# peterWon/GLoc3D

Hardware: AMD Instinct MI355X
Metric: localization queries/sec (kNN+top-20 reg), KITTI-00-sized DB (higher is better)
Workload: dtype f32

## Files before the change

gloc3d_amd/csrc/common.hip:

```cpp
#include "common.hpp"

namespace gloc {

char* err_buf() {
  static thread_local char buf[512] = {0};
  return buf;
}

void set_err(const char* fmt, ...) {
  va_list ap;
  va_start(ap, fmt);
  vsnprintf(err_buf(), 512, fmt, ap);
  va_end(ap);
}

int select_device(int device) {
  int n = 0;
  hipError_t e = hipGetDeviceCount(&n);
  if (e != hipSuccess || n <= 0) {
    set_err("no HIP device visible (%s): the gloc3d hot path has no CPU fallback",
            e == hipSuccess ? "device count 0" : hipGetErrorString(e));
    return GLOC_ERR_NODEVICE;
  }
  if (device < 0 || device >= n) {
    set_err("device ordinal %d out of range [0,%d)", device, n);
    return GLOC_ERR_INVALID;
  }
  hipDeviceProp_t prop;
  GLOC_HIP(hipGetDeviceProperties(&prop, device));
  if (strncmp(prop.gcnArchName, "gfx950", 6) != 0) {
    set_err("device %d is %s; this library is built for gfx950 (MI355X) only", device,
            prop.gcnArchName);
    return GLOC_ERR_NODEVICE;
  }
  GLOC_HIP(hipSetDevice(device));
  return GLOC_OK;
}

int DevBuf::ensure(size_t bytes, hipStream_t s, bool keep, size_t used) {
  if (bytes <= cap) return GLOC_OK;
  size_t ncap = cap ? cap : 256;
  while (ncap < bytes) ncap += ncap / 2 + 256;
  void* np = nullptr;
  GLOC_HIP(hipMalloc(&np, ncap));
  if (keep && p && used) {
    hipError_t e = hipMemcpyAsync(np, p, used, hipMemcpyDeviceToDevice, s);
    if (e == hipSuccess) e = hipStreamSynchronize(s);
    if (e != hipSuccess) {
      (void)hipFree(np);
      set_err("device buffer growth failed: %s", hipGetErrorString(e));
      return GLOC_ERR_HIP;
    }
  }
  if (p) GLOC_HIP(hipFree(p));
  p = np;
  cap = ncap;
  return GLOC_OK;
}

void DevBuf::release() {
  if (p) (void)hipFree(p);
  p = nullptr;
  cap = 0;
}

hipEvent_t Profiler::get_event() {
  if (!pool.empty()) {
    hipEvent_t e = pool.back();
    pool.pop_back();
    return e;
  }
  hipEvent_t e;
  (void)hipEventCreate(&e);
  return e;
}

void Profiler::begin(const char* name, hipStream_t s) {
  Family& f = fam[name];
  Span sp{get_event(), get_event()};
  (void)hipEventRecord(sp.a, s);
  f.open.push_back(sp);
}

void Profiler::end(const char* name, hipStream_t s) {
  Family& f = fam[name];
  if (f.open.empty()) return;
  (void)hipEventRecord(f.open.back().b, s);
  f.launches++;
  size_t live = 0;
  for (auto& kv : fam) live += kv.second.open.size();
  if (live > 8192) (void)collect(s);
}

int Profiler::collect(hipStream_t s) {
  GLOC_HIP(hipStreamSynchronize(s));
  for (auto& kv : fam) {
    for (Span& sp : kv.second.open) {
      float ms = 0.f;
      if (hipEventElapsedTime(&ms, sp.a, sp.b) == hipSuccess) kv.second.total_ms += ms;
      pool.push_back(sp.a);
      pool.push_back(sp.b);
    }
    kv.second.open.clear();
  }
  return GLOC_OK;
}

void Profiler::reset() {
  for (auto& kv : fam) {
    for (Span& sp : kv.second.open) {
      pool.push_back(sp.a);
      pool.push_back(sp.b);
    }
    kv.second.open.clear();
    kv.second.total_ms = 0;
    kv.second.launches = 0;
  }
}

void Profiler::destroy() {
  reset();
  for (hipEvent_t e : pool) (void)hipEventDestroy(e);
  pool.clear();
  fam.clear();
}

Handle::~Handle() {
  prof.destroy();
  if (own_stream) (void)hipStreamDestroy(own_stream);
}

int handle_open(Handle* h, int device) {
  h->device = device;
  hipError_t e = hipStreamCreateWithFlags(&h->own_stream, hipStreamNonBlocking);
  if (e != hipSuccess) {
    set_err("hipStreamCreate failed: %s", hipGetErrorString(e));
    return GLOC_ERR_HIP;
  }
  h->stream = h->own_stream;
  return GLOC_OK;
}

int handle_set_stream(Handle* h, void* hip_stream) {
  GLOC_TRY(handle_synchronize(h));
  h->stream = hip_stream ? static_cast<hipStream_t>(hip_stream) : h->own_stream;
  return GLOC_OK;
}

int handle_synchronize(Handle* h) {
  GLOC_REQUIRE(h, GLOC_ERR_INVALID, "handle is NULL");
  GLOC_HIP(hipSetDevice(h->device));
  GLOC_HIP(hipStreamSynchronize(h->stream));
  return GLOC_OK;
}

int handle_set_profile(Handle* h, int enable) {
  GLOC_REQUIRE(h, GLOC_ERR_INVALID, "handle is NULL");
  h->prof.enabled = enable != 0;
  return GLOC_OK;
}

int handle_profile(Handle* h, const char* kernel, double* total_ms, uint64_t* launches) {
  GLOC_REQUIRE(h && kernel, GLOC_ERR_INVALID, "NULL argument");
  GLOC_HIP(hipSetDevice(h->device));
  GLOC_TRY(h->prof.collect(h->stream));
  auto it = h->prof.fam.find(kernel);
  if (total_ms) *total_ms = it == h->prof.fam.end() ? 0.0 : it->second.total_ms;
// ... 26 lines not shown
```

gloc3d_amd/csrc/common.hpp:

```cpp
#pragma once
#include <hip/hip_runtime.h>

#include <cstdarg>
#include <cstdint>
#include <cstdio>
#include <cstring>
#include <map>
#include <new>
#include <string>
#include <type_traits>
#include <vector>

#include "../../include/gloc3d.h"

namespace gloc {

char* err_buf();
void set_err(const char* fmt, ...);

#define GLOC_HIP(expr)                                                                    \
  do {                                                                                    \
    hipError_t e_ = (expr);                                                               \
    if (e_ != hipSuccess) {                                                               \
      ::gloc::set_err("%s failed: %s (%s:%d)", #expr, hipGetErrorString(e_), __FILE__,    \
// ... 7 lines not shown
    if (!(cond)) {                     \
      ::gloc::set_err(__VA_ARGS__);    \
      return (code);                   \
    }                                  \
  } while (0)

#define GLOC_TRY(expr)            \
  do {                            \
    int rc_ = (expr);             \
    if (rc_ != GLOC_OK) return rc_; \
  } while (0)

int select_device(int device);

struct DevBuf {
  void* p = nullptr;
  size_t cap = 0;
  DevBuf() = default;
  DevBuf(const DevBuf&) = delete;
  DevBuf& operator=(const DevBuf&) = delete;
  DevBuf(DevBuf&& o) noexcept : p(o.p), cap(o.cap) { o.p = nullptr, o.cap = 0; }
  DevBuf& operator=(DevBuf&& o) noexcept {
    if (this != &o) {
      release();
      p = o.p, cap = o.cap;
      o.p = nullptr, o.cap = 0;
    }
    return *this;
  }
  ~DevBuf() { release(); }
  int ensure(size_t bytes, hipStream_t s, bool keep = false, size_t used = 0);
  void release();
  template <class T>
  T* as() const {
    return reinterpret_cast<T*>(p);
  }
};

static_assert(!std::is_copy_constructible<DevBuf>::value && !std::is_copy_assignable<DevBuf>::value,
              "a DevBuf has one owner: two copies would free the same memory");

struct Profiler {
  bool enabled = false;
  struct Span {
    hipEvent_t a, b;
  };
  struct Family {
    std::vector<Span> open;
    double total_ms = 0;
    uint64_t launches = 0;
  };
  std::map<std::string, Family> fam;
  std::vector<hipEvent_t> pool;
  hipEvent_t get_event();
  void begin(const char* name, hipStream_t s);
  void end(const char* name, hipStream_t s);
  int collect(hipStream_t s);
  void reset();
  void destroy();
};

struct ProfScope {
  Profiler& p;
  const char* name;
  hipStream_t s;
  ProfScope(Profiler& p_, const char* n, hipStream_t s_) : p(p_), name(n), s(s_) {
    if (p.enabled) p.begin(name, s);
  }
  ~ProfScope() {
    if (p.enabled) p.end(name, s);
  }
};

struct Handle {
  int device = 0;
  hipStream_t own_stream = nullptr, stream = nullptr;
  Profiler prof;
  Handle() = default;
  Handle(const Handle&) = delete;
  Handle& operator=(const Handle&) = delete;
  ~Handle();
};

int handle_open(Handle* h, int device);
int handle_set_stream(Handle* h, void* hip_stream);
int handle_synchronize(Handle* h);
int handle_set_profile(Handle* h, int enable);
int handle_profile(Handle* h, const char* kernel, double* total_ms, uint64_t* launches);
int handle_profile_reset(Handle* h);

template <class H>
int create_handle(int device, H** out) {
  GLOC_REQUIRE(out, GLOC_ERR_INVALID, "out is NULL");
  *out = nullptr;
  GLOC_TRY(select_device(device));
  H* h = new (std::nothrow) H();
  GLOC_REQUIRE(h, GLOC_ERR_NOMEM, "out of host memory");
  const int rc = handle_open(h, device);
  if (rc != GLOC_OK) {
    delete h;
    return rc;
  }
  *out = h;
  return GLOC_OK;
}

template <class H>
int destroy_handle(H* h) {
  if (!h) return GLOC_OK;
  (void)hipSetDevice(h->device);
  (void)hipStreamSynchronize(h->stream);
  delete h;
  return GLOC_OK;
}

template <class W>
int ensure_ws(W** slot) {
  if (!*slot) *slot = new (std::nothrow) W;
  GLOC_REQUIRE(*slot, GLOC_ERR_NOMEM, "host allocation failed");
  return GLOC_OK;
}

struct Staging {
// ... 15 lines not shown
```

gloc3d_amd/csrc/nn_compact.hpp:

```cpp
#pragma once
#include <hip/hip_runtime.h>
#include <stdint.h>

#include <type_traits>

#include "lane_ops.hpp"
#include "reg_kernels.hpp"

namespace gloc {
namespace reg {

typedef float f32x2 __attribute__((ext_vector_type(2)));

#define GPTR(T) const T __attribute__((address_space(1)))*
#define CPTR(T) const T __attribute__((address_space(4)))*
constexpr float NN_NEAR = 1.0e-6f;
constexpr float NN_LB_SCALE = 0.999998f;
#ifndef GLOC_NN_THIN_MIN
#define GLOC_NN_THIN_MIN 32
#endif
#ifdef GLOC_NN_MARKS
#define NN_MARK(n) asm volatile("; NN_MARK " n)
#else
#define NN_MARK(n)
// ... 1163 lines not shown
    static_assert(ACC_NV == 18, "16 scattered moments, the d2 sum, sum |p'|^2");
    static_assert(sizeof(double) * ACC_NV >= sizeof(float) * WAVE_PARTIAL_FLOATS, "a wave partial fits a partial's slot");
    float* out = reinterpret_cast<float*>(partials + ((size_t)job * n_part + gi) * ACC_NV);
#pragma unroll
    for (int k = 0; k < 8; ++k) mv[k] = exchange_add<32>(mv[k], mv[k + 8]);
#pragma unroll
    for (int k = 0; k < 4; ++k) mv[k] = exchange_add<16>(mv[k], mv[k + 4]);
    {
      const bool up = (lane & 8) != 0;
#pragma unroll
      for (int k = 0; k < 2; ++k) {
        const float keep = up ? mv[k + 2] : mv[k], send = up ? mv[k] : mv[k + 2];
        mv[k] = keep + xor_lane<8>(send);
      }
    }
    {
      const bool up = (lane & 4) != 0;
      const float keep = up ? mv[1] : mv[0], send = up ? mv[0] : mv[1];
      mv[0] = keep + xor_lane<4>(send);
    }
    float x = mv[0], y = mv[16];
    x += xor_lane<2>(x);
    x += xor_lane<1>(x);
    y = exchange_add<32>(y, pp);
    y = exchange_add<16>(y, y);
    y += xor_lane<8>(y);
    y += xor_lane<4>(y);
    y += xor_lane<2>(y);
    y += xor_lane<1>(y);
    if ((lane & 3) == 0) st_f32<CHAIN>(out + ((lane >> 2) & 15), x);
    if (lane == 0) {
      st_f32<CHAIN>(out + 16, y);
      st_f32<CHAIN>(out + 17, cen[0]);
      st_f32<CHAIN>(out + 18, cen[1]);
      st_f32<CHAIN>(out + 19, cen[2]);
    }
    if (lane == 32) st_f32<CHAIN>(out + 20, y);
  }
  NN_MARK("end");
}

#define NN_COMPACT_PARAMS                                                                                              \
  const Job *__restrict__ jobs, uint32_t n_jobs, uint32_t job_group, uint32_t n_wg, uint32_t subs,                     \
      const CandState *__restrict__ states, const uint32_t *prev_corr, uint32_t *corr, float *__restrict__ d2out,      \
      f32x4 *__restrict__ pairs, double *__restrict__ partials, uint32_t n_part, size_t ld, float gate2, NnSplit sp,   \
      NnHeavy hv, unsigned long long *__restrict__ stat_pairs
#define NN_COMPACT_ARGS jobs, n_jobs, job_group, n_wg, subs, states, prev_corr, corr, d2out, pairs, partials, n_part, ld, gate2, sp, hv, stat_pairs

template <int CS, bool PAIRS, bool SPLIT = false, bool WARM = false>
__global__ __launch_bounds__(64 * NN_WPB) void nn_compact_kernel(NN_COMPACT_PARAMS) {
  nn_compact_body<CS, PAIRS, SPLIT, WARM>(NnPos{blockIdx.z, blockIdx.x, blockIdx.y}, NN_COMPACT_ARGS);
}

template <int CS, bool PAIRS>
__global__ __launch_bounds__(64) void nn_compact_heavy_kernel(NN_COMPACT_PARAMS) {
  nn_compact_body<CS, PAIRS, true, false, true>(NnPos{0u, 0u, 0u}, NN_COMPACT_ARGS);
}

template <int CS>
__global__ __launch_bounds__(64 * NN_WPB) __attribute__((amdgpu_waves_per_eu(6, 6))) void nn_compact_split_warm_kernel(NN_COMPACT_PARAMS) {
  nn_compact_body<CS, false, true, true>(NnPos{blockIdx.z, blockIdx.x, blockIdx.y}, NN_COMPACT_ARGS);
}

template <int CS>
__global__ __launch_bounds__(64 * NN_WPB) __attribute__((amdgpu_waves_per_eu(6, 6))) void nn_chain_kernel(NN_COMPACT_PARAMS, NnChain ch) {
  static_assert(NN_WPB == 1, "a work-group is a wave: the roles and the arrival counts are per wave");
  const uint32_t b = blockIdx.x;
  const uint32_t pass = b / ch.pass_size, r1 = b - pass * ch.pass_size;
  const uint32_t grp = r1 / ch.grp_size, r2 = r1 - grp * ch.grp_size;
  const uint32_t n_search = job_group * n_wg;
  if (r2 >= n_search) {
    const uint32_t si = r2 - n_search, jl = si / NN_CHAIN_ROLES, role = si - jl * NN_CHAIN_ROLES;
    const uint32_t job = grp * ch.jobs_per_grp + jl;
    if (jl >= ch.jobs_per_grp || job >= n_jobs) return;
    const size_t cell = ((size_t)pass * n_jobs + job) * NN_CHAIN_PAD;
    if (role == NN_CHAIN_RED) {
      if (!chain_wait<false>(ch.done + cell, ch.expected, ch.err)) return;
      if ((threadIdx.x & 63) == 0) st_u32<true>(ch.go + cell, 1u);
    } else if (!chain_wait<false>(ch.go + cell, 1u, ch.err)) {
      return;
    }
    nn_compact_body<CS, false, true, true, false, true>(NnPos{0u, 0u, 0u, 1u + role, pass, job}, jobs, n_jobs, job_group, n_wg, subs, states,
                                                        corr, corr, d2out, pairs, partials, n_part, ld, gate2, sp, hv, stat_pairs, ch);
    return;
  }
  const uint32_t wgv = r2 / job_group, slot = r2 - wgv * job_group;
  uint32_t vin = slot;
  if ((job_group & 7u) == 0u) vin = (slot & ~7u) | ((slot - (slot >> 3) - grp) & 7u);
  const uint32_t vjob = grp * job_group + vin;
  if (vjob >= n_jobs * subs) return;
  const uint32_t job = vjob / subs;
  const size_t cell = ((size_t)pass * n_jobs + job) * NN_CHAIN_PAD;
  NnSplit spp = sp;
  if (pass > 0u) {
    if (!chain_wait<true>(ch.ready + cell, 2u, ch.err)) return;
    spp.plan = ch.planp + (size_t)(pass - 1u) * n_jobs * n_part;
    spp.helper = ch.helperp + (size_t)(pass - 1u) * n_jobs * sp.hx;
  }
  nn_compact_body<CS, false, true, true, false, true>(NnPos{grp, slot, wgv, 0u, pass, job}, jobs, n_jobs, job_group, n_wg, subs, states, corr, corr,
                                                      d2out, pairs, partials, n_part, ld, gate2, spp, hv, stat_pairs, ch);
  __builtin_amdgcn_s_waitcnt(0);
  asm volatile("" ::: "memory");
  if ((threadIdx.x & 63) == 0) (void)__hip_atomic_fetch_add(ch.done + cell, 1u, __ATOMIC_RELAXED, __HIP_MEMORY_SCOPE_AGENT);
}
#undef NN_COMPACT_PARAMS
#undef NN_COMPACT_ARGS
// ... 4 lines not shown
```

gloc3d_amd/csrc/reg.hip:

```cpp
#include <algorithm>
#include <cmath>
#include <vector>

#include "common.hpp"

#include "fpfh.hpp"
#include "ndt.hpp"
#include "nn_compact.hpp"
#include "gicp.hpp"
#include "p2l.hpp"
#include "pairgraph.hpp"
#include "reg_kernels.hpp"
#include "robust.hpp"
#include "scan_store.hpp"
#include "vgicp.hpp"

using namespace gloc;
using namespace gloc::reg;

struct gloc_reg : Handle {
  hipEvent_t done_ev = nullptr;
  gloc_scan_store* store = nullptr;
  gloc_scan_store* own_store = nullptr;
  DevBuf jobs, states;
// ... 167 lines not shown
  sp.thresh = h->nn_split_thresh_set || !chained ? h->nn_split_thresh : 85000u;
  return GLOC_OK;
}

int setup_heavy(gloc_reg* h, const BatchDims& bd, int cs) {
  h->heavy = NnHeavy{};
  if (h->nn_mode == 1 || cs != 2 || h->nn_heavy_thresh <= 0) return GLOC_OK;
  const size_t cap = std::min<size_t>((size_t)bd.n_jobs * 16, 16384), S = 64 * (size_t)cs;
  hipStream_t s = h->stream;
  auto keys_at = [](size_t c) { return (256 + c * 8 + c * 4 + 255) & ~(size_t)255; };
  if (cap > h->heavy_cap) {
    GLOC_TRY(h->heavy_buf.ensure(keys_at(cap) + 2 * cap * S * 8 + 256, s));
    GLOC_HIP(hipMemsetAsync(h->heavy_buf.p, 0, keys_at(cap), s));
    GLOC_HIP(hipMemsetAsync(h->heavy_buf.as<char>() + keys_at(cap), 0xFF, cap * S * 8, s));
    h->heavy_cap = cap;
  }
  char* b = h->heavy_buf.as<char>();
  NnHeavy& hv = h->heavy;
  hv.count = reinterpret_cast<uint32_t*>(b);
  hv.list = reinterpret_cast<uint32_t*>(b + 256);
  hv.ticket = reinterpret_cast<uint32_t*>(b + 256 + h->heavy_cap * 8);
  hv.skey = reinterpret_cast<unsigned long long*>(b + keys_at(h->heavy_cap));
  hv.hkey = hv.skey + h->heavy_cap * S;
  hv.cap = (uint32_t)cap;
  hv.thresh = (uint32_t)h->nn_heavy_thresh;
  return GLOC_OK;
}

void launch_order(const gloc_reg* h, uint32_t n_jobs, uint32_t& jg, uint32_t& subs) {
  subs = h->nn_sub_jobs > 0 ? (uint32_t)h->nn_sub_jobs : (n_jobs < 48 ? 8u : 1u);
  jg = (uint32_t)h->nn_job_group;
  if (h->nn_sub_jobs > 0 || h->nn_job_group_set || n_jobs >= 48) return;
  jg = 8u;
  subs = n_jobs % 4u == 0u ? 2u : (n_jobs % 2u == 0u ? 4u : 8u);
}

struct NnArgs {
  const WsView& v;
  const BatchDims& bd;
  uint32_t jg, n_wg, subs;
  float gate2;
  unsigned long long* stat_pairs;
};

template <auto KERNEL, typename... Chain>
void launch_compact(const NnArgs& a, dim3 grid, const uint32_t* prev_corr, bool pairs, NnHeavy hv, Chain... chain) {
  hipLaunchKernelGGL(KERNEL, grid, dim3(64 * NN_WPB), 0, a.v.s, a.v.jobs, a.v.n_jobs, a.jg, a.n_wg, a.subs, a.v.states, prev_corr,
                     a.v.corr, a.v.d2, a.v.pairs, pairs ? (double*)nullptr : a.v.partials, a.bd.n_part, a.bd.ld, a.gate2, a.v.split, hv,
                     a.stat_pairs, chain...);
}

template <int CS, bool PAIRS, bool WARM>
void launch_pass(const NnArgs& a, dim3 grid, const uint32_t* prev_corr, NnHeavy hv) {
  if (!a.v.split.hx) launch_compact<nn_compact_kernel<CS, PAIRS, false, WARM>>(a, grid, prev_corr, PAIRS, hv);
  else if constexpr (CS == 2 && !PAIRS && WARM) launch_compact<nn_compact_split_warm_kernel<2>>(a, grid, prev_corr, PAIRS, hv);
  else launch_compact<nn_compact_kernel<CS, PAIRS, true, WARM>>(a, grid, prev_corr, PAIRS, hv);
}

template <int CS>
void launch_kind(const NnArgs& a, dim3 grid, const uint32_t* prev_corr, NnHeavy hv, bool want_pairs, bool warm) {
  if (want_pairs) launch_pass<CS, true, false>(a, grid, prev_corr, hv);
  else if (warm) launch_pass<CS, false, true>(a, grid, prev_corr, hv);
  else launch_pass<CS, false, false>(a, grid, prev_corr, hv);
}

int launch_nn(gloc_reg* h, const BatchDims& bd, const WsView& v, bool warm, bool want_pairs, float gate2) {
  ProfScope ps(h->prof, "nn", v.s);
  Profiler no_prof;
  ProfScope ps_cold((want_pairs || !warm) ? h->prof : no_prof, "nn_cold", v.s);
  h->nn_launches++;
  if (h->nn_mode == 1) {
    dim3 grid((bd.max_src + 256 * NN_S - 1) / (256 * NN_S), v.n_jobs);
    hipLaunchKernelGGL(nn_kernel, grid, dim3(256), 0, v.s, v.jobs, v.states,
                       v.corr, v.d2, bd.ld);
    if (want_pairs)
      hipLaunchKernelGGL(gather_pairs_kernel, dim3((bd.max_src + 255) / 256, v.n_jobs), dim3(256), 0, v.s,
                         v.jobs, v.states, v.corr, bd.ld,
                         v.pairs);
  } else {
    const int cs = h->nn_src_per_lane;
    const bool cold = want_pairs || !warm;
    const NnHeavy hv = cold ? v.heavy : NnHeavy{};
    if (hv.cap) GLOC_HIP(hipMemsetAsync(hv.count, 0, 4, v.s));
    const uint32_t n_wg_job = (bd.max_groups + v.split.hx + NN_WPB - 1) / NN_WPB;
    uint32_t jg, subs;
    launch_order(h, v.n_jobs, jg, subs);
    const uint32_t n_slots = v.n_jobs * subs;
    const uint32_t n_wg = (n_wg_job + subs - 1) / subs;
    const unsigned grid = n_wg * jg * ((n_slots + jg - 1) / jg);
    GLOC_REQUIRE(n_wg <= 65535u && (n_slots + jg - 1) / jg <= 65535u, GLOC_ERR_INVALID,
                 "the culled search's grid: %u work-groups per job slot (scans above ~8 M points) or %u job groups exceed 65535", n_wg,
                 (n_slots + jg - 1) / jg);
    if (grid) {
      const NnArgs a{v, bd, jg, n_wg, subs, gate2, h->prof.enabled ? h->counters.as<unsigned long long>() : nullptr};
      const dim3 g3(jg, n_wg, (n_slots + jg - 1) / jg);
      const uint32_t* prev_corr = warm ? v.corr : nullptr;
      if (cs == 1) launch_kind<1>(a, g3, prev_corr, hv, want_pairs, warm);
      else if (cs == 2) launch_kind<2>(a, g3, prev_corr, hv, want_pairs, warm);
      else launch_kind<4>(a, g3, prev_corr, hv, want_pairs, warm);
      if (hv.cap) {
        const dim3 gh(hv.cap * NN_HEAVY_PARTS);
        if (want_pairs) launch_compact<nn_compact_heavy_kernel<2, true>>(a, gh, nullptr, true, hv);
        else launch_compact<nn_compact_heavy_kernel<2, false>>(a, gh, nullptr, false, hv);
      }
    }
  }
  GLOC_HIP(hipGetLastError());
  return GLOC_OK;
}

bool batch_chains(const gloc_reg* h, const BatchDims& bd, uint32_t hx, uint32_t warm_passes) {
  if (!h->nn_chain || h->chain_broken || h->nn_mode == 1 || h->nn_src_per_lane != 2 || h->prof.enabled || NN_WPB != 1) return false;
  if (hx == 0 || warm_passes < 2) return false;
  uint32_t jg, subs;
  launch_order(h, bd.n_jobs, jg, subs);
  if (bd.n_jobs >= 48 || (jg & 7u) || jg % subs) return false;
  if ((bd.n_part & 31u) || (hx & 31u)) return false;
  const uint32_t n_wg = ((bd.max_groups + hx + NN_WPB - 1) / NN_WPB + subs - 1) / subs;
  const uint32_t groups = (bd.n_jobs * subs + jg - 1) / jg;
  const uint64_t grp_size = ((uint64_t)jg * n_wg + (jg / subs) * NN_CHAIN_ROLES + 7) & ~7ull;
  return grp_size * groups * warm_passes < (1ull << 31);
}
// ... 102 lines not shown
  v.jobs = h->jobs.as<Job>();
  v.states = h->states.as<CandState>();
  v.partials = h->partials.as<double>();
  if (sp.search) {
    if (!h->counters.p) {
      GLOC_TRY(h->counters.ensure(8 * NN_STAT_SLOTS, s));
      GLOC_HIP(hipMemsetAsync(h->counters.p, 0, 8 * NN_STAT_SLOTS, s));
    }
    GLOC_TRY(h->corr.ensure(sizeof(uint32_t) * std::max<size_t>(bd.ld, 1) * n_jobs, s));
    GLOC_TRY(h->d2.ensure(sizeof(float) * std::max<size_t>(bd.ld, 1) * n_jobs, s));
    v.corr = h->corr.as<uint32_t>();
    v.d2 = h->d2.as<float>();
  }
  if (sp.pairs) {
    GLOC_TRY(h->pairs.ensure(sizeof(f32x4) * 2 * bd.ld * n_jobs, s));
    GLOC_TRY(h->Rt.ensure(sizeof(float) * 12 * sp.hyp * n_jobs, s));
    GLOC_TRY(h->valid.ensure(sizeof(uint32_t) * sp.hyp * n_jobs, s));
    GLOC_TRY(h->inliers.ensure(sizeof(uint32_t) * sp.hyp * n_jobs, s));
    v.pairs = h->pairs.as<f32x4>();
    v.Rt = h->Rt.as<float>();
    v.valid = h->valid.as<uint32_t>();
    v.inliers = h->inliers.as<uint32_t>();
    if (sp.alive) {
      GLOC_TRY(h->alive.ensure(sizeof(uint32_t) * (sp.hyp + 1) * n_jobs, s));
      v.a_idx = h->alive.as<uint32_t>();
      v.a_cnt = v.a_idx + sp.hyp * n_jobs;
    }
  }
  GLOC_HIP(hipMemcpyAsync(v.jobs, h->h_jobs, sizeof(Job) * n_jobs, hipMemcpyHostToDevice, s));
  GLOC_HIP(hipMemcpyAsync(v.states, h->h_states, sizeof(CandState) * n_jobs, hipMemcpyHostToDevice, s));
  b.chained = batch_chains(h, bd, sp.split_hx, sp.warm_passes);
  GLOC_TRY(setup_split(h, bd, cs, sp.split_hx, b.chained));
  if (sp.search) GLOC_TRY(setup_heavy(h, bd, cs));
  else h->heavy = NnHeavy{};
  v.split = h->split;
  v.heavy = h->heavy;
  if (sp.search) {
    h->last_ld = bd.ld;
    h->last_jobs = n_jobs;
  }
  return GLOC_OK;
}

uint32_t score_chunk_len(uint32_t n_jobs, uint32_t max_src) {
  static_assert(1024 % SC_STAGE == 0 && SC_CHUNK % SC_STAGE == 0, "whole tiles");
  return (size_t)n_jobs * ((max_src + SC_CHUNK - 1) / SC_CHUNK) >= 2048 ? (uint32_t)SC_CHUNK : 1024u;
}

uint32_t score_hpb(uint32_t len) { return len <= 16 ? 16u : (len <= 64 ? 64u : 256u); }

int enqueue_refit(gloc_reg* h, const BatchDims& bd, const WsView& v, float thr2, uint32_t nblocks) {
  const uint32_t n_jobs = v.n_jobs;
  {
    ProfScope ps(h->prof, "accum", v.s);
    hipLaunchKernelGGL(accum_kernel<1>, dim3(nblocks, n_jobs), dim3(ACC_THREADS), 0, v.s, v.jobs, v.states, v.corr, v.d2, v.pairs, bd.ld, thr2,
                       v.partials, bd.n_part);
    GLOC_HIP(hipGetLastError());
  }
  {
    ProfScope ps(h->prof, "solve", v.s);
    hipLaunchKernelGGL(solve_kernel<1>, dim3(v.split.hx ? 2 * n_jobs : n_jobs), dim3(SOLVE_THREADS), 0, v.s, v.partials, bd.n_part, false, v.jobs,
                       v.states, v.split, n_jobs);
    GLOC_HIP(hipGetLastError());
  }
  return GLOC_OK;
}

struct RansacRule {
  uint32_t iters;
  float inlier_thresh, min_inlier_ratio, confidence;
  uint64_t seed;
};

int enqueue_ransac(gloc_reg* h, const BatchDims& bd, const RansacRule& r, const WsView& v, uint32_t nblocks) {
  const uint32_t n_jobs = v.n_jobs;
  hipStream_t s = v.s;
  const uint32_t H = r.iters;
  const bool adaptive = r.confidence > 0.f && r.confidence < 1.f;
  uint32_t bounds[4] = {0u, 0u, 0u, 0u};
  int n_ph = 0;
  for (uint32_t b : {adaptive ? 16u : 256u, adaptive ? 64u : H, H})
    if (b <= H && b > bounds[n_ph]) bounds[++n_ph] = b;
  if (bounds[n_ph] < H) bounds[++n_ph] = H;
  GLOC_HIP(hipMemsetAsync(v.valid, 0, sizeof(uint32_t) * (size_t)H * n_jobs, s));
  GLOC_HIP(hipMemsetAsync(v.inliers, 0, sizeof(uint32_t) * (size_t)H * n_jobs, s));
  const float thr2 = r.inlier_thresh * r.inlier_thresh;
  const uint32_t chunk_len = score_chunk_len(n_jobs, bd.max_src);
  const unsigned cchunks = (bd.max_src + chunk_len - 1) / chunk_len;
  for (int ph = 0; ph < n_ph; ++ph) {
    const uint32_t h0 = bounds[ph], h1 = bounds[ph + 1], len = h1 - h0;
    const CandState* st = ph ? v.states : (const CandState*)nullptr;
    {
      ProfScope ps(h->prof, "ransac_hyp", s);
      hipLaunchKernelGGL(ransac_hyp_kernel, dim3((len + 127) / 128, n_jobs), dim3(128), 0, s, v.pairs, bd.ld,
                         v.jobs, r.seed, H, h0, h1, st, v.Rt, v.valid);
      GLOC_HIP(hipGetLastError());
    }
    ProfScope ps(h->prof, "ransac_score", s);
    const uint32_t hpb = score_hpb(len);
    const unsigned NP = 8;
    if (!adaptive && ph > 0 && len >= 512 && cchunks >= NP) {
      uint32_t* a_idx = v.a_idx;
      uint32_t* a_cnt = v.a_cnt;
      for (unsigned q = 0; q < NP; ++q) {
        const unsigned c0 = q * cchunks / NP, c1 = (q + 1) * cchunks / NP;
        hipLaunchKernelGGL(ransac_alive_kernel, dim3(n_jobs), dim3(1024), 0, s, v.inliers, v.valid,
                           H, h0, h1, v.jobs, v.states, (uint32_t)(c0 * chunk_len), a_idx, a_cnt);
        hipLaunchKernelGGL(ransac_score_kernel, dim3((len + 255) / 256, c1 - c0, n_jobs), dim3(256), 0, s,
                           v.pairs, bd.ld, v.jobs, H, h0, 256u, v.Rt,
                           v.valid, thr2, st, v.inliers, a_idx, a_cnt, (uint32_t)c0, chunk_len);
      }
    } else {
      hipLaunchKernelGGL(ransac_score_kernel, dim3((len + hpb - 1) / hpb, cchunks, n_jobs), dim3(256), 0, s,
                         v.pairs, bd.ld, v.jobs, H, h0, hpb, v.Rt,
                         v.valid, thr2, st, v.inliers, (const uint32_t*)nullptr,
                         (const uint32_t*)nullptr, 0u, chunk_len);
    }
    if (ph + 1 < n_ph)
      hipLaunchKernelGGL(ransac_scan_kernel<false>, dim3(n_jobs), dim3(64), 0, s, v.inliers,
                         v.valid, v.Rt, H, h0, h1, v.jobs, r.confidence,
                         r.min_inlier_ratio, v.states);
    else
      hipLaunchKernelGGL(ransac_scan_kernel<true>, dim3(n_jobs), dim3(64), 0, s, v.inliers,
                         v.valid, v.Rt, H, h0, h1, v.jobs, r.confidence,
                         r.min_inlier_ratio, v.states);
    GLOC_HIP(hipGetLastError());
  }
  return enqueue_refit(h, bd, v, thr2, nblocks);
}

int enqueue_pipeline(gloc_reg* h, const BatchDims& bd, const gloc_reg_params* prm, const WsView& v, bool can, bool any_tgt,
                     uint32_t nblocks, bool chained) {
  const uint32_t n_jobs = v.n_jobs;
  hipStream_t s = v.s;
  const bool culled = h->nn_mode != 1;
  const float gate2 = prm->max_corr_dist > 0.f ? prm->max_corr_dist * prm->max_corr_dist : 0.f;
  bool have_corr = false;

  if (can && any_tgt && prm->ransac_iters > 0) {
    GLOC_TRY(launch_nn(h, bd, v, false, true, 0.f));
    have_corr = true;
    GLOC_TRY(enqueue_ransac(h, bd, RansacRule{prm->ransac_iters, prm->inlier_thresh, prm->min_inlier_ratio, prm->ransac_confidence, prm->seed},
                            v, nblocks));
  }
  for (uint32_t it = 0; it < prm->icp_iters && can && any_tgt; ++it) {
    if (chained && have_corr) {
      GLOC_TRY(launch_nn_chain(h, bd, v, prm->icp_iters - it, gate2));
      break;
    }
    GLOC_TRY(launch_nn(h, bd, v, have_corr, false, gate2));
    have_corr = true;
    if (!culled) {
      ProfScope ps(h->prof, "accum", s);
      hipLaunchKernelGGL(accum_kernel<0>, dim3(nblocks, n_jobs), dim3(ACC_THREADS), 0, s, v.jobs,
                         v.states, v.corr, v.d2,
                         (const f32x4*)nullptr, bd.ld, gate2, v.partials, bd.n_part);
      GLOC_HIP(hipGetLastError());
    }
    {
      ProfScope ps(h->prof, "solve", s);
      hipLaunchKernelGGL(solve_kernel<0>, dim3(v.split.hx ? 2 * n_jobs : n_jobs), dim3(SOLVE_THREADS), 0, s, v.partials,
                         bd.n_part, culled, v.jobs, v.states, v.split, n_jobs);
      GLOC_HIP(hipGetLastError());
    }
  }
  return GLOC_OK;
}

int enqueue_jobs(gloc_reg* h, const std::vector<JobHost>& jh, const gloc_reg_params* prm) {
  const uint32_t n_jobs = (uint32_t)jh.size();
  if (n_jobs == 0) return GLOC_OK;
  const int cs = h->nn_src_per_lane;
  uint32_t max_src = 0;
  bool can = false, any_tgt = false;
  for (const JobHost& j : jh) {
    max_src = std::max<uint32_t>(max_src, (uint32_t)j.src.n);
    can |= j.src.n >= 3;
    any_tgt |= j.tgt.n >= 1;
  }
  const bool ransac = can && any_tgt && prm->ransac_iters > 0;
  const bool adaptive = prm->ransac_confidence > 0.f && prm->ransac_confidence < 1.f;
  const uint32_t warm_passes = !(can && any_tgt) ? 0u : (ransac ? prm->icp_iters : std::max<uint32_t>(prm->icp_iters, 1u) - 1u);
  BatchSpec spec = BatchSpec::searching(n_jobs, max_src, src_groups(max_src, cs));
  spec.pairs = ransac;
  spec.hyp = prm->ransac_iters;
  spec.alive = !adaptive;
  spec.split_hx = split_helpers(h, n_jobs);
  spec.warm_passes = warm_passes;
  Batch b;
  GLOC_TRY(open_batch(h, spec, &b, [&](Job* jd, CandState* st) {
    for (uint32_t c = 0; c < n_jobs; ++c) {
      const DevScan &s = jh[c].src, &t = jh[c].tgt;
      jd[c] = Job{s.idx.pts, s.order, s.idx.inv, t.xyz, t.idx, (uint32_t)s.n, src_groups(s.n, cs), jh[c].stream_id, 0u};
      init_state(st[c], jh[c].init_T, prm->ransac_iters);
      if (s.n < 3) st[c].frozen = 1;
    }
  }));
  hipStream_t s = h->stream;
  GLOC_TRY(enqueue_pipeline(h, b.bd, prm, b.v, can, any_tgt, b.nblocks, b.chained));
  GLOC_HIP(hipMemcpyAsync(h->h_states, h->states.p, sizeof(CandState) * n_jobs, hipMemcpyDeviceToHost, s));
  GLOC_HIP(hipEventRecord(h->done_ev, s));
  if (h->chain_in_batch) {
    h->retry_jobs.resize(sizeof(JobHost) * n_jobs);
    memcpy(h->retry_jobs.data(), jh.data(), sizeof(JobHost) * n_jobs);
    h->retry_T.assign((size_t)16 * n_jobs, 0.f);
    for (uint32_t c = 0; c < n_jobs; ++c)
      if (jh[c].init_T) memcpy(&h->retry_T[(size_t)16 * c], jh[c].init_T, sizeof(float) * 16);
    h->retry_prm = *prm;
  }
  return GLOC_OK;
}

int collect_jobs(gloc_reg* h, uint32_t n_jobs, const size_t* n_src_of, float max_rmse, float max_final_step, float* out_T,
                 float* out_rmse, uint32_t* out_inliers, int* out_ok) {
// ... 1284 lines not shown
```

gloc3d_amd/csrc/reg_kernels.hpp:

```cpp
#pragma once
#include <hip/hip_runtime.h>
#include <stdint.h>

#include "math3.hpp"
#include "lane_ops.hpp"
#include "scan_index.hpp"
#include "synth_kernels.hpp"

namespace gloc {
namespace reg {


struct Job {
  const f32x4* src_pts;
  const uint32_t* src_order;
  const uint32_t* src_inv;
  const float* tgt_xyz;
  ScanIndexDev tgt;
  uint32_t n_src, n_groups;
  uint32_t cand_id;
  uint32_t pad_;
};

struct NnSplit {
// ... 570 lines not shown
      const f32x4 p = J.src_pts[i];
      xform(T, p.x, p.y, p.z, px, py, pz);
      const uint32_t j = corr[(size_t)cand * ld + i];
      if (j >= J.tgt.n) continue;
      const f32x4 t = J.tgt.pts[j];
      qx = t.x; qy = t.y; qz = t.z;
      const float d2 = d2in[(size_t)cand * ld + i];
      v[16] += (double)d2;
      use = !(gate2 > 0.f) || (d2 < gate2);
    } else {
      const f32x4 p = pairs[((size_t)cand * ld + i) * 2 + 0];
      const f32x4 q = pairs[((size_t)cand * ld + i) * 2 + 1];
      px = p.x; py = p.y; pz = p.z;
      qx = q.x; qy = q.y; qz = q.z;
      if (qx >= 0.5f * NN_FAR) continue;
      v[16] += (double)dist2(px, py, pz, qx, qy, qz);
      float x, y, z;
      xform(T, px, py, pz, x, y, z);
      use = dist2(x, y, z, qx, qy, qz) < gate2;
    }
    if (use) {
      const double P[3] = {(double)px, (double)py, (double)pz};
      const double Q[3] = {(double)qx, (double)qy, (double)qz};
      v[0] += 1.0;
#pragma unroll
      for (int a = 0; a < 3; ++a) {
        v[1 + a] += P[a];
        v[4 + a] += Q[a];
#pragma unroll
        for (int b = 0; b < 3; ++b) v[7 + 3 * a + b] += P[a] * Q[b];
      }
      v[17] += (P[0] * P[0] + P[1] * P[1]) + P[2] * P[2];
    }
  }
  const int lane = threadIdx.x & 63, w = threadIdx.x >> 6;
#pragma unroll
  for (int k = 0; k < ACC_NV; ++k) {
    double x = v[k];
    for (int o = 32; o > 0; o >>= 1) x += __shfl_xor(x, o);
    if (lane == 0) red[w][k] = x;
  }
  __syncthreads();
  if (threadIdx.x < ACC_NV) {
    double s = 0.0;
    for (int ww = 0; ww < ACC_THREADS / 64; ++ww) s += red[ww][threadIdx.x];
    partials[((size_t)cand * n_part + blockIdx.x) * ACC_NV + threadIdx.x] = s;
  }
}

constexpr int WAVE_PARTIAL_FLOATS = 21;
constexpr int SOLVE_R = 56;
constexpr int SOLVE_THREADS = 1024;
static_assert(SOLVE_R * ACC_NV <= SOLVE_THREADS, "a thread per (stride class, moment)");

template <bool COH>
__device__ __forceinline__ uint32_t ld_u32(const uint32_t* p) {
  if constexpr (COH) return __hip_atomic_load(p, __ATOMIC_RELAXED, __HIP_MEMORY_SCOPE_AGENT);
  else return *p;
}
template <bool COH>
__device__ __forceinline__ void st_u32(uint32_t* p, uint32_t v) {
  if constexpr (COH) __hip_atomic_store(p, v, __ATOMIC_RELAXED, __HIP_MEMORY_SCOPE_AGENT);
  else *p = v;
}
template <bool COH>
__device__ __forceinline__ unsigned long long ld_u64(const unsigned long long* p) {
  if constexpr (COH) return __hip_atomic_load(p, __ATOMIC_RELAXED, __HIP_MEMORY_SCOPE_AGENT);
  else return *p;
}
template <bool COH>
__device__ __forceinline__ void st_u64(unsigned long long* p, unsigned long long v) {
  if constexpr (COH) __hip_atomic_store(p, v, __ATOMIC_RELAXED, __HIP_MEMORY_SCOPE_AGENT);
  else *p = v;
}
template <bool COH>
__device__ __forceinline__ double ld_f64(const double* p) {
  return __builtin_bit_cast(double, ld_u64<COH>(reinterpret_cast<const unsigned long long*>(p)));
}
template <bool COH>
__device__ __forceinline__ void st_f64(double* p, double v) {
  st_u64<COH>(reinterpret_cast<unsigned long long*>(p), __builtin_bit_cast(unsigned long long, v));
}
template <bool COH>
__device__ __forceinline__ float ld_f32(const float* p) {
  return __uint_as_float(ld_u32<COH>(reinterpret_cast<const uint32_t*>(p)));
}
template <bool COH>
__device__ __forceinline__ void st_f32(float* p, float v) {
  st_u32<COH>(reinterpret_cast<uint32_t*>(p), __float_as_uint(v));
}

__device__ __forceinline__ void add_wave_partial(const float* f , double* v ) {
  const double n = (double)f[0];
  const double c[3] = {(double)f[17], (double)f[18], (double)f[19]};
  v[0] += n;
  v[16] += (double)f[16];
  v[17] += ((double)f[20] + 2.0 * ((c[0] * (double)f[1] + c[1] * (double)f[2]) + c[2] * (double)f[3])) +
           n * ((c[0] * c[0] + c[1] * c[1]) + c[2] * c[2]);
#pragma unroll
  for (int a = 0; a < 3; ++a) {
    v[1 + a] += (double)f[1 + a] + n * c[a];
    v[4 + a] += (double)f[4 + a] + n * c[a];
#pragma unroll
    for (int b = 0; b < 3; ++b)
      v[7 + 3 * a + b] += (((double)f[7 + 3 * a + b] + c[a] * (double)f[4 + b]) + (double)f[1 + a] * c[b]) + n * (c[a] * c[b]);
  }
// ... 111 lines not shown
        work[g] = 0;
      }
      const unsigned long long b2 = __ballot(parts == 2), b4 = __ballot(parts == 4), b8 = __ballot(parts == 8);
      const unsigned long long below = (1ull << lane) - 1ull;
      my_parts[t] = parts;
      my_pre[t] = parts >= 4 ? 4u * (uint32_t)__popcll(b4 & below) + 8u * (uint32_t)__popcll(b8 & below) : 2u * (uint32_t)__popcll(b2 & below);
      my_gpre[t] = parts >= 4 ? (uint32_t)__popcll((b4 | b8) & below) : (uint32_t)__popcll(b2 & below);
      if (lane == 0) {
        cnt_h[t][w] = 4u * (uint32_t)__popcll(b4) + 8u * (uint32_t)__popcll(b8);
        cnt_l[t][w] = 2u * (uint32_t)__popcll(b2);
        grp_h[t][w] = (uint32_t)__popcll(b4 | b8);
        grp_l[t][w] = (uint32_t)__popcll(b2);
      }
    }
    for (uint32_t e = (uint32_t)tid; e < sp.hx; e += SOLVE_THREADS) helper[e] = NN_NO_HELPER;
    __syncthreads();
    uint32_t tot_h = 0, tot_gh = 0;
    for (uint32_t t = 0; t < n_tiles; ++t)
      for (int i = 0; i < SOLVE_THREADS / 64; ++i) {
        tot_h += cnt_h[t][i];
        tot_gh += grp_h[t][i];
      }
    uint32_t run_h = 0, run_l = tot_h, run_gh = 0, run_gl = tot_gh;
#pragma unroll
    for (int t = 0; t < PLAN_TILES; ++t) {
      if ((uint32_t)t >= n_tiles) continue;
      uint32_t bh = run_h, bl = run_l, bgh = run_gh, bgl = run_gl;
      for (int i = 0; i < SOLVE_THREADS / 64; ++i) {
        if (i < w) {
          bh += cnt_h[t][i];
          bl += cnt_l[t][i];
          bgh += grp_h[t][i];
          bgl += grp_l[t][i];
        }
        run_h += cnt_h[t][i];
        run_l += cnt_l[t][i];
        run_gh += grp_h[t][i];
        run_gl += grp_l[t][i];
      }
      const uint32_t g = (uint32_t)t * SOLVE_THREADS + (uint32_t)tid, parts = my_parts[t];
      if (g >= ng) continue;
      const uint32_t first = (parts >= 4 ? bh : bl) + my_pre[t], hid = (parts >= 4 ? bgh : bgl) + my_gpre[t];
      uint32_t word = 0;
      if (parts > 1 && first + parts <= sp.hx) {
        for (uint32_t p = 0; p < parts; ++p) helper[first + p] = g | (p << 20) | (parts << 24);
        word = (hid << 8) | parts;
      }
      plan[g] = word;
    }
    for (uint32_t g = ng + (uint32_t)tid; g < jobs[cand].n_groups; g += SOLVE_THREADS) plan[g] = 0;
    return;
  }
  const int cand = blockIdx.x;
  const uint32_t cnt = per_group ? jobs[cand].n_groups
                                 : (jobs[cand].n_src + ACC_PER_BLOCK - 1) / ACC_PER_BLOCK;
  if (per_group) {
    static_assert(SOLVE_THREADS / 64 <= SOLVE_R, "a row of sub[][] per wave");
    const float* base = reinterpret_cast<const float*>(partials + (size_t)cand * n_part * ACC_NV);
    double v[ACC_NV];
#pragma unroll
    for (int k = 0; k < ACC_NV; ++k) v[k] = 0.0;
    for (uint32_t g = (uint32_t)tid; g < cnt; g += SOLVE_THREADS) {
      typedef float f32x2_ __attribute__((ext_vector_type(2)));
      const f32x2_* f2 = reinterpret_cast<const f32x2_*>(base + (size_t)g * (2 * ACC_NV));
      float f[WAVE_PARTIAL_FLOATS + 1];
#pragma unroll
      for (int i = 0; i < (WAVE_PARTIAL_FLOATS + 1) / 2; ++i) {
        const f32x2_ t = f2[i];
        f[2 * i] = t.x;
        f[2 * i + 1] = t.y;
      }
      add_wave_partial(f, v);
    }
#pragma unroll
    for (int k = 0; k < ACC_NV; ++k) {
      double x = v[k];
      x += xor_lane<32>(x);
      x += xor_lane<16>(x);
      x += xor_lane<8>(x);
      x += xor_lane<4>(x);
      x += xor_lane<2>(x);
      x += xor_lane<1>(x);
      v[k] = x;
    }
    if ((tid & 63) == 0) {
#pragma unroll
      for (int k = 0; k < ACC_NV; ++k) sub[tid >> 6][k] = v[k];
    }
  } else if (tid < SOLVE_R * ACC_NV) {
    const int k = tid % ACC_NV, r = tid / ACC_NV;
    double acc = 0.0;
    uint32_t b = (uint32_t)r;
    const double* pp = partials + (size_t)cand * n_part * ACC_NV + k;
    for (; b + 3 * SOLVE_R < cnt; b += 4 * SOLVE_R) {
      const double v0 = pp[(size_t)b * ACC_NV], v1 = pp[(size_t)(b + SOLVE_R) * ACC_NV];
      const double v2 = pp[(size_t)(b + 2 * SOLVE_R) * ACC_NV], v3 = pp[(size_t)(b + 3 * SOLVE_R) * ACC_NV];
      acc += v0; acc += v1; acc += v2; acc += v3;
    }
    for (; b < cnt; b += SOLVE_R) acc += pp[(size_t)b * ACC_NV];
    sub[r][k] = acc;
  }
  __syncthreads();
  if (tid < ACC_NV) {
    double acc = 0.0;
    const int rows = per_group ? SOLVE_THREADS / 64 : SOLVE_R;
    for (int r = 0; r < rows; ++r) acc += sub[r][tid];
    tot[tid] = acc;
  }
  __syncthreads();
  if (tid != 0) return;
  double v[ACC_NV];
#pragma unroll
  for (int k = 0; k < ACC_NV; ++k) v[k] = tot[k];
  solve_compose<MODE, false>(v, &states[cand], states[cand].Td, (uint32_t)states[cand].frozen);
}

}
}
```

Measured before the change: 611.2.

## Shrink non-split solve blocks, add cold NN kernel variant, share profiler events

```diff
diff --git a/gloc3d_amd/csrc/common.hip b/gloc3d_amd/csrc/common.hip
--- a/gloc3d_amd/csrc/common.hip
+++ b/gloc3d_amd/csrc/common.hip
@@ -1,4 +1,6 @@
 #include "common.hpp"
+
+#include <algorithm>
 
 namespace gloc {
 
@@ -75,44 +77,66 @@
   return e;
 }
 
-void Profiler::begin(const char* name, hipStream_t s) {
+void Profiler::begin(const char* name, hipStream_t s, bool joined) {
   Family& f = fam[name];
-  Span sp{get_event(), get_event()};
-  (void)hipEventRecord(sp.a, s);
+  Span sp;
+  if (joined && tail && tail_s == s) {
+    sp.a = tail;
+  } else {
+    sp.a = get_event();
+    (void)hipEventRecord(sp.a, s);
+  }
+  sp.b = get_event();
+  tail = nullptr;
   f.open.push_back(sp);
 }
 
-void Profiler::end(const char* name, hipStream_t s) {
+void Profiler::end(const char* name, hipStream_t s, const char* also) {
   Family& f = fam[name];
   if (f.open.empty()) return;
-  (void)hipEventRecord(f.open.back().b, s);
+  const Span sp = f.open.back();
+  (void)hipEventRecord(sp.b, s);
+  tail = sp.b;
+  tail_s = s;
   f.launches++;
+  if (also) {
+    Family& g = fam[also];
+    g.open.push_back(sp);
+    g.launches++;
+  }
   size_t live = 0;
   for (auto& kv : fam) live += kv.second.open.size();
   if (live > 8192) (void)collect(s);
 }
 
-int Profiler::collect(hipStream_t s) {
-  GLOC_HIP(hipStreamSynchronize(s));
-  for (auto& kv : fam) {
-    for (Span& sp : kv.second.open) {
-      float ms = 0.f;
-      if (hipEventElapsedTime(&ms, sp.a, sp.b) == hipSuccess) kv.second.total_ms += ms;
-      pool.push_back(sp.a);
-      pool.push_back(sp.b);
-    }
-    kv.second.open.clear();
-  }
-  return GLOC_OK;
-}
-
-void Profiler::reset() {
+void Profiler::release_open() {
+  const size_t first = pool.size();
   for (auto& kv : fam) {
     for (Span& sp : kv.second.open) {
       pool.push_back(sp.a);
       pool.push_back(sp.b);
     }
     kv.second.open.clear();
+  }
+  std::sort(pool.begin() + first, pool.end());
+  pool.erase(std::unique(pool.begin() + first, pool.end()), pool.end());
+  tail = nullptr;
+}
+
+int Profiler::collect(hipStream_t s) {
+  GLOC_HIP(hipStreamSynchronize(s));
+  for (auto& kv : fam)
+    for (Span& sp : kv.second.open) {
+      float ms = 0.f;
+      if (hipEventElapsedTime(&ms, sp.a, sp.b) == hipSuccess) kv.second.total_ms += ms;
+    }
+  release_open();
+  return GLOC_OK;
+}
+
+void Profiler::reset() {
+  release_open();
+  for (auto& kv : fam) {
     kv.second.total_ms = 0;
     kv.second.launches = 0;
   }
diff --git a/gloc3d_amd/csrc/common.hpp b/gloc3d_amd/csrc/common.hpp
--- a/gloc3d_amd/csrc/common.hpp
+++ b/gloc3d_amd/csrc/common.hpp
@@ -83,23 +83,28 @@
   };
   std::map<std::string, Family> fam;
   std::vector<hipEvent_t> pool;
+  hipEvent_t tail = nullptr;
+  hipStream_t tail_s = nullptr;
   hipEvent_t get_event();
-  void begin(const char* name, hipStream_t s);
-  void end(const char* name, hipStream_t s);
+  void begin(const char* name, hipStream_t s, bool joined = false);
+  void end(const char* name, hipStream_t s, const char* also = nullptr);
   int collect(hipStream_t s);
+  void release_open();
   void reset();
   void destroy();
 };
 
 struct ProfScope {
+  enum Join { Apart, Joined };
   Profiler& p;
   const char* name;
   hipStream_t s;
-  ProfScope(Profiler& p_, const char* n, hipStream_t s_) : p(p_), name(n), s(s_) {
-    if (p.enabled) p.begin(name, s);
+  const char* also;
+  ProfScope(Profiler& p_, const char* n, hipStream_t s_, Join j = Apart, const char* also_ = nullptr) : p(p_), name(n), s(s_), also(also_) {
+    if (p.enabled) p.begin(name, s, j == Joined);
   }
   ~ProfScope() {
-    if (p.enabled) p.end(name, s);
+    if (p.enabled) p.end(name, s, also);
   }
 };
 
diff --git a/gloc3d_amd/csrc/nn_compact.hpp b/gloc3d_amd/csrc/nn_compact.hpp
--- a/gloc3d_amd/csrc/nn_compact.hpp
+++ b/gloc3d_amd/csrc/nn_compact.hpp
@@ -1239,6 +1239,11 @@
   nn_compact_body<CS, PAIRS, SPLIT, WARM>(NnPos{blockIdx.z, blockIdx.x, blockIdx.y}, NN_COMPACT_ARGS);
 }
 
+template <bool PAIRS>
+__global__ __launch_bounds__(64 * NN_WPB) __attribute__((amdgpu_waves_per_eu(6, 6))) void nn_compact_cold_kernel(NN_COMPACT_PARAMS) {
+  nn_compact_body<2, PAIRS, false, false>(NnPos{blockIdx.z, blockIdx.x, blockIdx.y}, NN_COMPACT_ARGS);
+}
+
 template <int CS, bool PAIRS>
 __global__ __launch_bounds__(64) void nn_compact_heavy_kernel(NN_COMPACT_PARAMS) {
   nn_compact_body<CS, PAIRS, true, false, true>(NnPos{0u, 0u, 0u}, NN_COMPACT_ARGS);
diff --git a/gloc3d_amd/csrc/reg.hip b/gloc3d_amd/csrc/reg.hip
--- a/gloc3d_amd/csrc/reg.hip
+++ b/gloc3d_amd/csrc/reg.hip
@@ -243,7 +243,10 @@
 
 template <int CS, bool PAIRS, bool WARM>
 void launch_pass(const NnArgs& a, dim3 grid, const uint32_t* prev_corr, NnHeavy hv) {
-  if (!a.v.split.hx) launch_compact<nn_compact_kernel<CS, PAIRS, false, WARM>>(a, grid, prev_corr, PAIRS, hv);
+  if (!a.v.split.hx) {
+    if constexpr (CS == 2 && !WARM) launch_compact<nn_compact_cold_kernel<PAIRS>>(a, grid, prev_corr, PAIRS, hv);
+    else launch_compact<nn_compact_kernel<CS, PAIRS, false, WARM>>(a, grid, prev_corr, PAIRS, hv);
+  }
   else if constexpr (CS == 2 && !PAIRS && WARM) launch_compact<nn_compact_split_warm_kernel<2>>(a, grid, prev_corr, PAIRS, hv);
   else launch_compact<nn_compact_kernel<CS, PAIRS, true, WARM>>(a, grid, prev_corr, PAIRS, hv);
 }
@@ -255,10 +258,8 @@
   else launch_pass<CS, false, false>(a, grid, prev_corr, hv);
 }
 
-int launch_nn(gloc_reg* h, const BatchDims& bd, const WsView& v, bool warm, bool want_pairs, float gate2) {
-  ProfScope ps(h->prof, "nn", v.s);
-  Profiler no_prof;
-  ProfScope ps_cold((want_pairs || !warm) ? h->prof : no_prof, "nn_cold", v.s);
+int launch_nn(gloc_reg* h, const BatchDims& bd, const WsView& v, bool warm, bool want_pairs, float gate2, ProfScope::Join join = ProfScope::Apart) {
+  ProfScope ps(h->prof, "nn", v.s, join, (want_pairs || !warm) ? "nn_cold" : nullptr);
   h->nn_launches++;
   if (h->nn_mode == 1) {
     dim3 grid((bd.max_src + 256 * NN_S - 1) / (256 * NN_S), v.n_jobs);
@@ -467,14 +468,14 @@
 int enqueue_refit(gloc_reg* h, const BatchDims& bd, const WsView& v, float thr2, uint32_t nblocks) {
   const uint32_t n_jobs = v.n_jobs;
   {
-    ProfScope ps(h->prof, "accum", v.s);
+    ProfScope ps(h->prof, "accum", v.s, ProfScope::Joined);
     hipLaunchKernelGGL(accum_kernel<1>, dim3(nblocks, n_jobs), dim3(ACC_THREADS), 0, v.s, v.jobs, v.states, v.corr, v.d2, v.pairs, bd.ld, thr2,
                        v.partials, bd.n_part);
     GLOC_HIP(hipGetLastError());
   }
   {
-    ProfScope ps(h->prof, "solve", v.s);
-    hipLaunchKernelGGL(solve_kernel<1>, dim3(v.split.hx ? 2 * n_jobs : n_jobs), dim3(SOLVE_THREADS), 0, v.s, v.partials, bd.n_part, false, v.jobs,
+    ProfScope ps(h->prof, "solve", v.s, ProfScope::Joined);
+    hipLaunchKernelGGL(solve_kernel<1>, dim3(v.split.hx ? 2 * n_jobs : n_jobs), dim3(v.split.hx ? SOLVE_THREADS : SOLVE_THREADS_LIGHT), 0, v.s, v.partials, bd.n_part, false, v.jobs,
                        v.states, v.split, n_jobs);
     GLOC_HIP(hipGetLastError());
   }
@@ -506,12 +507,12 @@
     const uint32_t h0 = bounds[ph], h1 = bounds[ph + 1], len = h1 - h0;
     const CandState* st = ph ? v.states : (const CandState*)nullptr;
     {
-      ProfScope ps(h->prof, "ransac_hyp", s);
+      ProfScope ps(h->prof, "ransac_hyp", s, ph ? ProfScope::Joined : ProfScope::Apart);
       hipLaunchKernelGGL(ransac_hyp_kernel, dim3((len + 127) / 128, n_jobs), dim3(128), 0, s, v.pairs, bd.ld,
                          v.jobs, r.seed, H, h0, h1, st, v.Rt, v.valid);
       GLOC_HIP(hipGetLastError());
     }
-    ProfScope ps(h->prof, "ransac_score", s);
+    ProfScope ps(h->prof, "ransac_score", s, ProfScope::Joined);
     const uint32_t hpb = score_hpb(len);
     const unsigned NP = 8;
     if (!adaptive && ph > 0 && len >= 512 && cchunks >= NP) {
@@ -563,18 +564,18 @@
       GLOC_TRY(launch_nn_chain(h, bd, v, prm->icp_iters - it, gate2));
       break;
     }
-    GLOC_TRY(launch_nn(h, bd, v, have_corr, false, gate2));
+    GLOC_TRY(launch_nn(h, bd, v, have_corr, false, gate2, have_corr ? ProfScope::Joined : ProfScope::Apart));
     have_corr = true;
     if (!culled) {
-      ProfScope ps(h->prof, "accum", s);
+      ProfScope ps(h->prof, "accum", s, ProfScope::Joined);
       hipLaunchKernelGGL(accum_kernel<0>, dim3(nblocks, n_jobs), dim3(ACC_THREADS), 0, s, v.jobs,
                          v.states, v.corr, v.d2,
                          (const f32x4*)nullptr, bd.ld, gate2, v.partials, bd.n_part);
       GLOC_HIP(hipGetLastError());
     }
     {
-      ProfScope ps(h->prof, "solve", s);
-      hipLaunchKernelGGL(solve_kernel<0>, dim3(v.split.hx ? 2 * n_jobs : n_jobs), dim3(SOLVE_THREADS), 0, s, v.partials,
+      ProfScope ps(h->prof, "solve", s, ProfScope::Joined);
+      hipLaunchKernelGGL(solve_kernel<0>, dim3(v.split.hx ? 2 * n_jobs : n_jobs), dim3(v.split.hx ? SOLVE_THREADS : SOLVE_THREADS_LIGHT), 0, s, v.partials,
                          bd.n_part, culled, v.jobs, v.states, v.split, n_jobs);
       GLOC_HIP(hipGetLastError());
     }
diff --git a/gloc3d_amd/csrc/reg_kernels.hpp b/gloc3d_amd/csrc/reg_kernels.hpp
--- a/gloc3d_amd/csrc/reg_kernels.hpp
+++ b/gloc3d_amd/csrc/reg_kernels.hpp
@@ -646,6 +646,8 @@
 constexpr int SOLVE_R = 56;
 constexpr int SOLVE_THREADS = 1024;
 static_assert(SOLVE_R * ACC_NV <= SOLVE_THREADS, "a thread per (stride class, moment)");
+constexpr int SOLVE_THREADS_LIGHT = 256;
+static_assert(SOLVE_THREADS_LIGHT % 64 == 0 && SOLVE_THREADS % SOLVE_THREADS_LIGHT == 0 && SOLVE_THREADS_LIGHT >= 64, "whole waves, whole turns");
 
 template <bool COH>
 __device__ __forceinline__ uint32_t ld_u32(const uint32_t* p) {
@@ -863,43 +865,47 @@
     return;
   }
   const int cand = blockIdx.x;
+  const int nthr = (int)blockDim.x;
   const uint32_t cnt = per_group ? jobs[cand].n_groups
                                  : (jobs[cand].n_src + ACC_PER_BLOCK - 1) / ACC_PER_BLOCK;
   if (per_group) {
     static_assert(SOLVE_THREADS / 64 <= SOLVE_R, "a row of sub[][] per wave");
     const float* base = reinterpret_cast<const float*>(partials + (size_t)cand * n_part * ACC_NV);
-    double v[ACC_NV];
-#pragma unroll
-    for (int k = 0; k < ACC_NV; ++k) v[k] = 0.0;
-    for (uint32_t g = (uint32_t)tid; g < cnt; g += SOLVE_THREADS) {
-      typedef float f32x2_ __attribute__((ext_vector_type(2)));
-      const f32x2_* f2 = reinterpret_cast<const f32x2_*>(base + (size_t)g * (2 * ACC_NV));
-      float f[WAVE_PARTIAL_FLOATS + 1];
-#pragma unroll
-      for (int i = 0; i < (WAVE_PARTIAL_FLOATS + 1) / 2; ++i) {
-        const f32x2_ t = f2[i];
-        f[2 * i] = t.x;
-        f[2 * i + 1] = t.y;
-      }
-      add_wave_partial(f, v);
-    }
-#pragma unroll
-    for (int k = 0; k < ACC_NV; ++k) {
-      double x = v[k];
-      x += xor_lane<32>(x);
-      x += xor_lane<16>(x);
-      x += xor_lane<8>(x);
-      x += xor_lane<4>(x);
-      x += xor_lane<2>(x);
-      x += xor_lane<1>(x);
-      v[k] = x;
-    }
-    if ((tid & 63) == 0) {
-#pragma unroll
-      for (int k = 0; k < ACC_NV; ++k) sub[tid >> 6][k] = v[k];
-    }
-  } else if (tid < SOLVE_R * ACC_NV) {
-    const int k = tid % ACC_NV, r = tid / ACC_NV;
+    const int lane = tid & 63, n_waves = nthr >> 6;
+    for (int rw = __builtin_amdgcn_readfirstlane(tid >> 6); rw < SOLVE_THREADS / 64; rw += n_waves) {
+      double v[ACC_NV];
+#pragma unroll
+      for (int k = 0; k < ACC_NV; ++k) v[k] = 0.0;
+      for (uint32_t g = (uint32_t)(rw * 64 + lane); g < cnt; g += SOLVE_THREADS) {
+        typedef float f32x2_ __attribute__((ext_vector_type(2)));
+        const f32x2_* f2 = reinterpret_cast<const f32x2_*>(base + (size_t)g * (2 * ACC_NV));
+        float f[WAVE_PARTIAL_FLOATS + 1];
+#pragma unroll
+        for (int i = 0; i < (WAVE_PARTIAL_FLOATS + 1) / 2; ++i) {
+          const f32x2_ t = f2[i];
+          f[2 * i] = t.x;
+          f[2 * i + 1] = t.y;
+        }
+        add_wave_partial(f, v);
+      }
+#pragma unroll
+      for (int k = 0; k < ACC_NV; ++k) {
+        double x = v[k];
+        x += xor_lane<32>(x);
+        x += xor_lane<16>(x);
+        x += xor_lane<8>(x);
+        x += xor_lane<4>(x);
+        x += xor_lane<2>(x);
+        x += xor_lane<1>(x);
+        v[k] = x;
+      }
+      if (lane == 0) {
+#pragma unroll
+        for (int k = 0; k < ACC_NV; ++k) sub[rw][k] = v[k];
+      }
+    }
+  } else for (int t = tid; t < SOLVE_R * ACC_NV; t += nthr) {
+    const int k = t % ACC_NV, r = t / ACC_NV;
     double acc = 0.0;
     uint32_t b = (uint32_t)r;
     const double* pp = partials + (size_t)cand * n_part * ACC_NV + k;
```

Measured after the change: 619.1 (median of 6 runs). 1.01x the previous value.
